# showlab/EgoVLP

Hardware: NVIDIA H100
Metric: clips/sec, 16-frame TimeSformer-B + DistilBERT + EgoNCE training step (higher is better)
Workload: dtype bf16

## Files before the change

egovlp_b200/csrc/attention.cu:

```cuda
#include <stdlib.h>

#include "common.cuh"
#include "egovlp_b200.h"

namespace egovlp {

bool space_attn_wgmma_supported(int N);
int space_attn_fwd_wgmma(const void* qkv, void* out, float* lse, float* cls_part, int B, int T, int N, int H,
                         cudaStream_t st);

namespace {

constexpr int HD = 64;
constexpr int ROW_BYTES = 128;
constexpr float LOG2E = 1.4426950408889634f;

struct Geom {
  int B, H, T, N, S, D;
  int mode;
  int PG;
  int G;
  int NP;
  int NPAD;
  int gsize;
};

__device__ __forceinline__ uint32_t sw_addr(uint32_t base, int row, int chunk) {
  return base + row * ROW_BYTES + ((chunk ^ (row & 7)) << 4);
}
__device__ __forceinline__ void ldsm_x4(uint32_t addr, uint32_t (&r)[4]) {
  asm volatile("ldmatrix.sync.aligned.m8n8.x4.shared.b16 {%0,%1,%2,%3}, [%4];"
               : "=r"(r[0]), "=r"(r[1]), "=r"(r[2]), "=r"(r[3]) : "r"(addr));
}
__device__ __forceinline__ void ldsm_x4_t(uint32_t addr, uint32_t (&r)[4]) {
  asm volatile("ldmatrix.sync.aligned.m8n8.x4.trans.shared.b16 {%0,%1,%2,%3}, [%4];"
               : "=r"(r[0]), "=r"(r[1]), "=r"(r[2]), "=r"(r[3]) : "r"(addr));
}
__device__ __forceinline__ void mma_bf16(float (&c)[4], const uint32_t (&a)[4], uint32_t b0, uint32_t b1) {
  asm volatile("mma.sync.aligned.m16n8k16.row.col.f32.bf16.bf16.f32 {%0,%1,%2,%3}, {%4,%5,%6,%7}, {%8,%9}, {%0,%1,%2,%3};"
               : "+f"(c[0]), "+f"(c[1]), "+f"(c[2]), "+f"(c[3])
               : "r"(a[0]), "r"(a[1]), "r"(a[2]), "r"(a[3]), "r"(b0), "r"(b1));
}
__device__ __forceinline__ void load_a_frag(uint32_t tile, int r0, int kk, int lane, uint32_t (&f)[4]) {
  ldsm_x4(sw_addr(tile, r0 + (lane & 7) + ((lane >> 3) & 1) * 8, kk * 2 + (lane >> 4)), f);
}
__device__ __forceinline__ void load_b_frag_nk(uint32_t tile, int n0, int kk, int lane, uint32_t (&f)[4]) {
  ldsm_x4(sw_addr(tile, n0 + (lane & 7) + (lane >> 4) * 8, kk * 2 + ((lane >> 3) & 1)), f);
}
__device__ __forceinline__ void load_b_frag_kn(uint32_t tile, int k0, int dp, int lane, uint32_t (&f)[4]) {
  ldsm_x4_t(sw_addr(tile, k0 + (lane & 7) + ((lane >> 3) & 1) * 8, dp * 2 + (lane >> 4)), f);
}

__device__ __forceinline__ int row_token(const Geom& G, int g, int r) {
  if (r == G.NP) return 0;
  if (r > G.NP) return -1;
  if (G.mode == 1) return 1 + g * G.N + r;
  const int j = r / G.T, f = r - j * G.T, n = g * G.PG + j;
  return n < G.N ? 1 + f * G.N + n : -1;
}

template <int RT>
__device__ __forceinline__ int row_token_x(const Geom& G, int g, int r, int sh) {
  if (RT == 0) return row_token(G, g, r);
  if (r == G.NP) return 0;
  if (r > G.NP) return -1;
  if (RT == 1) return 1 + g * G.N + r;
  const int n = g * G.PG + (r >> sh);
  return n < G.N ? 1 + (r & ((1 << sh) - 1)) * G.N + n : -1;
}

struct Smem {
  uint32_t q, k, v, dout;
  short* gid;
  float* lse;
  float* delta;
  uint32_t stage;
  uint32_t bar;
};

__device__ __forceinline__ bool pair_valid(int gq, int gk, bool first_group) {
  if (gq >= 0) return gk == gq || gk == -2;
  if (gq == -2) return gk >= 0 || (gk == -2 && first_group);
  return false;
}

__device__ __forceinline__ void tile_window(const Geom& G, int r0, int& lo, int& hi) {
  if (r0 <= G.NP && G.NP < r0 + 16) { lo = 0; hi = G.NP; return; }
  if (r0 > G.NP) { lo = 0; hi = 0; return; }
  lo = (r0 / G.gsize) * G.gsize;
  hi = min(G.NP, ((r0 + 15) / G.gsize + 1) * G.gsize);
}
__device__ __forceinline__ bool span_active(const Geom& G, int lo, int hi, int c0, int width) {
// ... 1038 lines not shown


}
}

using namespace egovlp;

extern "C" long long egovlp_divided_attn_workspace_floats(int B, int T, int N, int H, int mode) {
  Geom G;
  if (make_geom(G, B, T, N, H, mode)) return -1;
  return (long long)B * H * G.G * 4 * 66;
}

extern "C" int egovlp_divided_attn_fwd(const void* qkv, void* out, float* lse, float* cls_part, int B, int T, int N,
                                       int H, int mode, void* stream) {
  EGOVLP_CHECK_ARG(qkv && out && lse && cls_part, "divided_attn_fwd: null pointer");
  EGOVLP_CHECK_ARG(B > 0 && T > 0 && N > 0 && H > 0 && (mode == 0 || mode == 1), "divided_attn_fwd: bad shape");
  Geom G;
  if (make_geom(G, B, T, N, H, mode)) { set_last_error("divided_attn: unsupported geometry T=%d N=%d", T, N); return EGOVLP_ERR_UNSUPPORTED; }
  CUtensorMap tm;
  int rc = make_group_tmap(&tm, qkv, G, 3 * H);
  if (rc) return rc;
  cudaStream_t st = reinterpret_cast<cudaStream_t>(stream);
  const bf16* q = reinterpret_cast<const bf16*>(qkv);
  bf16* o = reinterpret_cast<bf16*>(out);
  const int grid = B * H * G.G;
#define LAUNCH_FWD(KERN, W, ...)                                                                              \
  do {                                                                                                        \
    const size_t smem = attn_smem_bytes(G, false, W, generic || mode == 1);                                   \
    EGOVLP_CHECK_CUDA(cudaFuncSetAttribute(KERN, cudaFuncAttributeMaxDynamicSharedMemorySize, (int)smem));    \
    KERN<<<grid, W * 32, smem, st>>>(tm, q, o, lse, cls_part, G, ##__VA_ARGS__);                              \
  } while (0)
  const bool generic = force_generic() || (mode == 0 && !time_fast_ok(G));
  if (!generic && mode == 1 && space_attn_wgmma_supported(N)) {
    rc = space_attn_fwd_wgmma(qkv, out, lse, cls_part, B, T, N, H, st);
    if (rc) return rc;
  } else if (generic) {
    if (G.NPAD > 128) LAUNCH_FWD((divided_attn_fwd_kernel<7, 2>), 7);
    else LAUNCH_FWD((divided_attn_fwd_kernel<4, 3>), 4);
  } else if (mode == 1) {
    if (G.NPAD > 128) LAUNCH_FWD((fast_attn_fwd_kernel<false, 7, 2>), 7, 0);
    else LAUNCH_FWD((fast_attn_fwd_kernel<false, 4, 3>), 4, 0);
  } else {
    LAUNCH_FWD((fast_attn_fwd_kernel<true, 4, 4>), 4, time_shift(G));
  }
#undef LAUNCH_FWD
  EGOVLP_CHECK_LAUNCH();
  const int BH = B * H;
  const int parts = (!generic && mode == 0) ? 4 : 1;
  cls_merge_kernel<<<(BH + 3) / 4, 128, 0, st>>>(cls_part, o, lse, BH, H, G.G * parts, G.S, G.D);
  EGOVLP_CHECK_LAUNCH();
  return EGOVLP_OK;
}

extern "C" int egovlp_divided_attn_bwd(const void* qkv, const void* out, const void* dout, const float* lse,
                                       void* dqkv, float* dcls_ws, int B, int T, int N, int H, int mode,
                                       float q_scale, void* stream) {
  EGOVLP_CHECK_ARG(qkv && out && dout && lse && dqkv && dcls_ws, "divided_attn_bwd: null pointer");
  EGOVLP_CHECK_ARG(B > 0 && T > 0 && N > 0 && H > 0 && (mode == 0 || mode == 1), "divided_attn_bwd: bad shape");
  Geom G;
  if (make_geom(G, B, T, N, H, mode)) { set_last_error("divided_attn: unsupported geometry T=%d N=%d", T, N); return EGOVLP_ERR_UNSUPPORTED; }
  CUtensorMap tmq, tmd;
  int rc = make_group_tmap(&tmq, qkv, G, 3 * H);
  if (rc) return rc;
  rc = make_group_tmap(&tmd, dout, G, H);
  if (rc) return rc;
  cudaStream_t st = reinterpret_cast<cudaStream_t>(stream);
  EGOVLP_CHECK_CUDA(cudaMemsetAsync(dcls_ws, 0, (size_t)B * H * 3 * HD * sizeof(float), st));
  const bf16* q = reinterpret_cast<const bf16*>(qkv);
  const bf16* o = reinterpret_cast<const bf16*>(out);
  const bf16* d_o = reinterpret_cast<const bf16*>(dout);
  bf16* dq = reinterpret_cast<bf16*>(dqkv);
  const int grid = B * H * G.G;
#define LAUNCH_BWD(KERN, W, ...)                                                                              \
  do {                                                                                                        \
    const size_t smem = attn_smem_bytes(G, true, W);                                                          \
    EGOVLP_CHECK_CUDA(cudaFuncSetAttribute(KERN, cudaFuncAttributeMaxDynamicSharedMemorySize, (int)smem));    \
    KERN<<<grid, W * 32, smem, st>>>(tmq, tmd, q, o, d_o, lse, dq, dcls_ws, q_scale, G, ##__VA_ARGS__);       \
  } while (0)
  const bool generic = force_generic() || (mode == 0 && !time_fast_ok(G));
  if (generic) {
    if (G.NPAD > 128) LAUNCH_BWD((divided_attn_bwd_kernel<7, 2>), 7);
    else LAUNCH_BWD((divided_attn_bwd_kernel<4, 3>), 4);
  } else if (mode == 1) {
    if (G.NPAD > 128) LAUNCH_BWD((fast_attn_bwd_kernel<false, 7, 2>), 7, 0);
    else LAUNCH_BWD((fast_attn_bwd_kernel<false, 4, 3>), 4, 0);
  } else {
    const char* we = getenv("EGOVLP_ATTN_TIME_BWD_WARPS");
    const bool w8 = we && we[0] == '8';
    if (w8) LAUNCH_BWD((fast_attn_bwd_kernel<true, 8, 2>), 8, time_shift(G));
    else LAUNCH_BWD((fast_attn_bwd_kernel<true, 4, 3>), 4, time_shift(G));
  }
#undef LAUNCH_BWD
  EGOVLP_CHECK_LAUNCH();
  const int n = B * H * 3 * HD;
  cls_grad_finalize_kernel<<<(n + 255) / 256, 256, 0, st>>>(dcls_ws, reinterpret_cast<bf16*>(dqkv), B, H, G.S, G.D, q_scale);
  EGOVLP_CHECK_LAUNCH();
  return EGOVLP_OK;
}
```

egovlp_b200/csrc/attention_wgmma.cu:

```cuda
#include <stdlib.h>

#include "common.cuh"
#include "egovlp_b200.h"

namespace egovlp {
namespace {

constexpr int HD = 64;
constexpr int ROWB = 128;
constexpr int QROWS = 256;
constexpr int KROWS = 208;
constexpr int Q_BYTES = QROWS * ROWB, KV_BYTES = KROWS * ROWB;
constexpr int SMEM_BYTES = Q_BYTES + 2 * KV_BYTES + 1024  + 64 ;
constexpr float LOG2E = 1.4426950408889634f;

struct SpaceGeom {
  int H, T, N, S, D;
};

__device__ __forceinline__ void wgmma_m64n208k16_ss(float (&d)[104], uint64_t adesc, uint64_t bdesc, int scale_d) {
  asm volatile(
      "{\n\t.reg .pred p;\n\t"
      "setp.ne.b32 p, %106, 0;\n\t"
      "wgmma.mma_async.sync.aligned.m64n208k16.f32.bf16.bf16 "
      "{%0,%1,%2,%3,%4,%5,%6,%7,%8,%9,%10,%11,%12,%13,%14,%15,%16,%17,%18,%19,%20,%21,%22,%23,%24,%25,%26,%27,%28,%29,%30,%31,"
      "%32,%33,%34,%35,%36,%37,%38,%39,%40,%41,%42,%43,%44,%45,%46,%47,%48,%49,%50,%51,%52,%53,%54,%55,%56,%57,%58,%59,%60,%61,%62,%63,"
      "%64,%65,%66,%67,%68,%69,%70,%71,%72,%73,%74,%75,%76,%77,%78,%79,%80,%81,%82,%83,%84,%85,%86,%87,%88,%89,%90,%91,%92,%93,%94,%95,"
      "%96,%97,%98,%99,%100,%101,%102,%103}, "
      "%104, %105, p, 1, 1, 0, 0;\n\t}"
      : "+f"(d[0]), "+f"(d[1]), "+f"(d[2]), "+f"(d[3]), "+f"(d[4]), "+f"(d[5]), "+f"(d[6]), "+f"(d[7]),
        "+f"(d[8]), "+f"(d[9]), "+f"(d[10]), "+f"(d[11]), "+f"(d[12]), "+f"(d[13]), "+f"(d[14]), "+f"(d[15]),
        "+f"(d[16]), "+f"(d[17]), "+f"(d[18]), "+f"(d[19]), "+f"(d[20]), "+f"(d[21]), "+f"(d[22]), "+f"(d[23]),
        "+f"(d[24]), "+f"(d[25]), "+f"(d[26]), "+f"(d[27]), "+f"(d[28]), "+f"(d[29]), "+f"(d[30]), "+f"(d[31]),
        "+f"(d[32]), "+f"(d[33]), "+f"(d[34]), "+f"(d[35]), "+f"(d[36]), "+f"(d[37]), "+f"(d[38]), "+f"(d[39]),
        "+f"(d[40]), "+f"(d[41]), "+f"(d[42]), "+f"(d[43]), "+f"(d[44]), "+f"(d[45]), "+f"(d[46]), "+f"(d[47]),
        "+f"(d[48]), "+f"(d[49]), "+f"(d[50]), "+f"(d[51]), "+f"(d[52]), "+f"(d[53]), "+f"(d[54]), "+f"(d[55]),
        "+f"(d[56]), "+f"(d[57]), "+f"(d[58]), "+f"(d[59]), "+f"(d[60]), "+f"(d[61]), "+f"(d[62]), "+f"(d[63]),
        "+f"(d[64]), "+f"(d[65]), "+f"(d[66]), "+f"(d[67]), "+f"(d[68]), "+f"(d[69]), "+f"(d[70]), "+f"(d[71]),
        "+f"(d[72]), "+f"(d[73]), "+f"(d[74]), "+f"(d[75]), "+f"(d[76]), "+f"(d[77]), "+f"(d[78]), "+f"(d[79]),
        "+f"(d[80]), "+f"(d[81]), "+f"(d[82]), "+f"(d[83]), "+f"(d[84]), "+f"(d[85]), "+f"(d[86]), "+f"(d[87]),
        "+f"(d[88]), "+f"(d[89]), "+f"(d[90]), "+f"(d[91]), "+f"(d[92]), "+f"(d[93]), "+f"(d[94]), "+f"(d[95]),
        "+f"(d[96]), "+f"(d[97]), "+f"(d[98]), "+f"(d[99]), "+f"(d[100]), "+f"(d[101]), "+f"(d[102]), "+f"(d[103])
      : "l"(adesc), "l"(bdesc), "r"(scale_d));
}
__device__ __forceinline__ void wgmma_m64n64k16_rs(float (&d)[32], uint32_t a0, uint32_t a1, uint32_t a2, uint32_t a3,
                                                  uint64_t bdesc, int scale_d) {
  asm volatile(
      "{\n\t.reg .pred p;\n\t"
      "setp.ne.b32 p, %37, 0;\n\t"
      "wgmma.mma_async.sync.aligned.m64n64k16.f32.bf16.bf16 "
      "{%0,%1,%2,%3,%4,%5,%6,%7,%8,%9,%10,%11,%12,%13,%14,%15,%16,%17,%18,%19,%20,%21,%22,%23,%24,%25,%26,%27,%28,%29,%30,%31}, "
      "{%32, %33, %34, %35}, %36, p, 1, 1, 1;\n\t}"
      : "+f"(d[0]), "+f"(d[1]), "+f"(d[2]), "+f"(d[3]), "+f"(d[4]), "+f"(d[5]), "+f"(d[6]), "+f"(d[7]),
        "+f"(d[8]), "+f"(d[9]), "+f"(d[10]), "+f"(d[11]), "+f"(d[12]), "+f"(d[13]), "+f"(d[14]), "+f"(d[15]),
        "+f"(d[16]), "+f"(d[17]), "+f"(d[18]), "+f"(d[19]), "+f"(d[20]), "+f"(d[21]), "+f"(d[22]), "+f"(d[23]),
        "+f"(d[24]), "+f"(d[25]), "+f"(d[26]), "+f"(d[27]), "+f"(d[28]), "+f"(d[29]), "+f"(d[30]), "+f"(d[31])
      : "r"(a0), "r"(a1), "r"(a2), "r"(a3), "l"(bdesc), "r"(scale_d));
}

__global__ void __launch_bounds__(256, 1)
space_attn_fwd_wgmma_kernel(const __grid_constant__ CUtensorMap tm_rows, const __grid_constant__ CUtensorMap tm_cls,
                            bf16* __restrict__ out, float* __restrict__ lse_out, float* __restrict__ cls_part, SpaceGeom G) {
  extern __shared__ uint8_t smem_raw[];
  const uint32_t base = (smem_u32(smem_raw) + 1023u) & ~1023u;
  uint8_t* gen = smem_raw + (base - smem_u32(smem_raw));
  const uint32_t sQ = base, sK = base + Q_BYTES, sV = sK + KV_BYTES, bar = sV + KV_BYTES;
  const int g = blockIdx.x;
  const int f = g % G.T, h = (g / G.T) % G.H, b = g / (G.T * G.H);
  const int NK = G.N + 1;

  for (int i = threadIdx.x; i < (Q_BYTES + 2 * KV_BYTES) / 16; i += blockDim.x)
    *reinterpret_cast<uint4*>(gen + 16 * i) = make_uint4(0, 0, 0, 0);
  fence_proxy_async_smem();
  if (threadIdx.x == 0) {
    mbar_init(bar, 1);
    fence_mbar_init();
  }
  __syncthreads();
  if (threadIdx.x == 0) {
    mbar_expect_tx(bar, 3u * (uint32_t)NK * ROWB);
#pragma unroll
    for (int w = 0; w < 3; ++w) {
      const uint32_t dst = w == 0 ? sQ : (w == 1 ? sK : sV);
      tma_load_4d(dst, &tm_rows, bar, 0, 1 + f * G.N, w * G.H + h, b);
      tma_load_4d(dst + G.N * ROWB, &tm_cls, bar, 0, 0, w * G.H + h, b);
    }
  }
  mbar_wait_nocall(bar, 0);

  const int wg = threadIdx.x >> 7, wq = (threadIdx.x >> 5) & 3, lane = threadIdx.x & 31;
  const int gq = lane >> 2, c = lane & 3;
  for (int t = wg; t < QROWS / 64; t += 2) {
    if (t * 64 > G.N) break;
    float s[KROWS / 2];
    wgmma_fence_regs(s);
    wgmma_fence();
#pragma unroll
    for (int kk = 0; kk < HD / 16; ++kk)
      wgmma_m64n208k16_ss(s, make_smem_desc_sw128(sQ + t * 64 * ROWB + kk * 32, 16, 1024),
                          make_smem_desc_sw128(sK + kk * 32, 16, 1024), kk > 0);
    wgmma_commit();
    wgmma_wait<0>();
    wgmma_fence_regs(s);
    const int r0 = t * 64 + wq * 16 + gq;
    float mx[2], sum[2];
#pragma unroll
    for (int h2 = 0; h2 < 2; ++h2) {
      const int vis = (r0 + 8 * h2 == G.N && f != 0) ? G.N : NK;
      float m = -INFINITY;
#pragma unroll
      for (int j = 0; j < KROWS / 8; ++j)
#pragma unroll
        for (int e = 0; e < 2; ++e) {
          float& v = s[4 * j + 2 * h2 + e];
          if (8 * j + 2 * c + e >= vis) v = -INFINITY;
          m = fmaxf(m, v);
        }
      m = fmaxf(m, __shfl_xor_sync(0xffffffffu, m, 1));
      mx[h2] = fmaxf(m, __shfl_xor_sync(0xffffffffu, m, 2));
    }
    uint32_t p[KROWS / 4];
#pragma unroll
    for (int h2 = 0; h2 < 2; ++h2) {
      const float nms = -mx[h2] * LOG2E;
      float acc = 0.f;
#pragma unroll
      for (int j = 0; j < KROWS / 8; ++j) {
        const float e0 = exp2f(fmaf(s[4 * j + 2 * h2], LOG2E, nms));
        const float e1 = exp2f(fmaf(s[4 * j + 2 * h2 + 1], LOG2E, nms));
        acc += e0 + e1;
        p[2 * j + h2] = pack_bf16x2(e0, e1);
      }
      acc += __shfl_xor_sync(0xffffffffu, acc, 1);
      sum[h2] = acc + __shfl_xor_sync(0xffffffffu, acc, 2);
    }
    float o[HD / 2];
    wgmma_fence_regs(o);
    wgmma_fence();
#pragma unroll
    for (int kk = 0; kk < KROWS / 16; ++kk)
      wgmma_m64n64k16_rs(o, p[4 * kk], p[4 * kk + 1], p[4 * kk + 2], p[4 * kk + 3],
                         make_smem_desc_sw128(sV + kk * 16 * ROWB, 8192, 1024), kk > 0);
    wgmma_commit();
    wgmma_wait<0>();
    wgmma_fence_regs(o);
#pragma unroll
    for (int h2 = 0; h2 < 2; ++h2) {
      const int row = r0 + 8 * h2;
      if (row < G.N) {
        const float inv = 1.f / sum[h2];
        const long long tok = (long long)b * G.S + 1 + f * G.N + row;
        bf16* dst = out + tok * G.D + h * HD + 2 * c;
#pragma unroll
        for (int j = 0; j < HD / 8; ++j)
          *reinterpret_cast<uint32_t*>(dst + 8 * j) = pack_bf16x2(o[4 * j + 2 * h2] * inv, o[4 * j + 2 * h2 + 1] * inv);
        if (c == 0) lse_out[((long long)(b * G.H + h)) * G.S + 1 + f * G.N + row] = mx[h2] + logf(sum[h2]);
      } else if (row == G.N) {
        float* dst = cls_part + (((long long)(b * G.H + h)) * G.T + f) * 66;
#pragma unroll
        for (int j = 0; j < HD / 8; ++j) {
          dst[8 * j + 2 * c] = o[4 * j + 2 * h2];
          dst[8 * j + 2 * c + 1] = o[4 * j + 2 * h2 + 1];
        }
        if (c == 0) { dst[64] = mx[h2]; dst[65] = sum[h2]; }
      }
    }
  }
}

}

bool space_attn_wgmma_supported(int N) {
  const char* e = getenv("EGOVLP_ATTN_TC");
  if (!(e && e[0] == '1')) return false;
  return N + 1 > 128 && N + 1 <= KROWS;
}

int space_attn_fwd_wgmma(const void* qkv, void* out, float* lse, float* cls_part, int B, int T, int N, int H,
                         cudaStream_t st) {
  SpaceGeom G;
  G.H = H; G.T = T; G.N = N; G.S = 1 + T * N; G.D = H * HD;
  const uint64_t W = 3ull * G.D;
  const uint64_t dims[4] = {HD, (uint64_t)G.S, (uint64_t)(3 * H), (uint64_t)B};
  const uint64_t strides[4] = {1, W, HD, (uint64_t)G.S * W};
  const uint32_t box_rows[4] = {HD, (uint32_t)N, 1, 1};
  const uint32_t box_cls[4] = {HD, 1, 1, 1};
  CUtensorMap tm_rows, tm_cls;
  int rc = make_tmap_nd_bf16(&tm_rows, qkv, 4, dims, strides, box_rows, true);
  if (rc) return rc;
  rc = make_tmap_nd_bf16(&tm_cls, qkv, 4, dims, strides, box_cls, true);
  if (rc) return rc;
  static bool attr = false;
  if (!attr) {
    EGOVLP_CHECK_CUDA(cudaFuncSetAttribute(space_attn_fwd_wgmma_kernel, cudaFuncAttributeMaxDynamicSharedMemorySize,
                                           SMEM_BYTES));
    attr = true;
  }
  space_attn_fwd_wgmma_kernel<<<B * H * T, 256, SMEM_BYTES, st>>>(tm_rows, tm_cls, reinterpret_cast<bf16*>(out), lse,
                                                                   cls_part, G);
  EGOVLP_CHECK_LAUNCH();
  return EGOVLP_OK;
}

}
```

egovlp_b200/csrc/common.cuh:

```cuda
#pragma once
#include <cuda.h>
#include <cuda_bf16.h>
#include <cuda_runtime.h>
#include <stdint.h>
#include <stdio.h>

#define EGOVLP_OK 0
#define EGOVLP_ERR_ARG (-1)
#define EGOVLP_ERR_CUDA (-2)
#define EGOVLP_ERR_UNSUPPORTED (-3)

namespace egovlp {

typedef __nv_bfloat16 bf16;

void set_last_error(const char* fmt, ...);

#define EGOVLP_CHECK_ARG(cond, ...)                                   \
  do {                                                                \
    if (!(cond)) {                                                    \
      ::egovlp::set_last_error(__VA_ARGS__);                          \
      return EGOVLP_ERR_ARG;                                          \
    }                                                                 \
  } while (0)
// ... 67 lines not shown
}
__device__ __forceinline__ unsigned long long dropout_key(unsigned long long seed, uint32_t site) {
  return seed ^ (0x9E3779B97F4A7C15ull * (unsigned long long)(site + 1));
}
__device__ __forceinline__ uint32_t dropout_threshold(float p) {
  const double t = (double)p * 4294967296.0;
  return t >= 4294967295.0 ? 0xFFFFFFFFu : (uint32_t)t;
}

__device__ __forceinline__ void mbar_init(uint32_t bar, uint32_t count) {
  asm volatile("mbarrier.init.shared::cta.b64 [%0], %1;" ::"r"(bar), "r"(count));
}
__device__ __forceinline__ void fence_mbar_init() {
  asm volatile("fence.mbarrier_init.release.cluster;" ::: "memory");
}
__device__ __forceinline__ void mbar_expect_tx(uint32_t bar, uint32_t bytes) {
  asm volatile("mbarrier.arrive.expect_tx.shared::cta.b64 _, [%0], %1;" ::"r"(bar), "r"(bytes) : "memory");
}
__device__ __forceinline__ void mbar_arrive(uint32_t bar) {
  asm volatile("mbarrier.arrive.shared::cta.b64 _, [%0];" ::"r"(bar) : "memory");
}
__device__ __forceinline__ uint32_t mbar_try_wait(uint32_t bar, uint32_t parity) {
  uint32_t ok;
  asm volatile(
      "{\n\t.reg .pred p;\n\t"
      "mbarrier.try_wait.parity.shared::cta.b64 p, [%1], %2;\n\t"
      "selp.u32 %0, 1, 0, p;\n\t}"
      : "=r"(ok)
      : "r"(bar), "r"(parity)
      : "memory");
  return ok;
}
__device__ __forceinline__ void mbar_wait(uint32_t bar, uint32_t parity) {
  if (mbar_try_wait(bar, parity)) return;
  const long long t0 = clock64();
  while (!mbar_try_wait(bar, parity)) {
    if (clock64() - t0 > 4000000000LL) {
      printf("egovlp: mbarrier timeout block %d thread %d bar %u parity %u\n", blockIdx.x, threadIdx.x, bar, parity);
      __trap();
    }
  }
}

__device__ __forceinline__ void mbar_wait_nocall(uint32_t bar, uint32_t parity) {
  if (mbar_try_wait(bar, parity)) return;
  const long long t0 = clock64();
  for (;;) {
#pragma unroll 1
    for (int i = 0; i < 1024; ++i)
      if (mbar_try_wait(bar, parity)) return;
    if (clock64() - t0 > 4000000000LL) __trap();
  }
}

__device__ __forceinline__ void tma_prefetch_desc(const CUtensorMap* m) {
  asm volatile("prefetch.tensormap [%0];" ::"l"(reinterpret_cast<uint64_t>(m)) : "memory");
}
__device__ __forceinline__ void tma_load_2d(uint32_t dst, const CUtensorMap* m, uint32_t bar, int c0, int c1) {
  asm volatile(
      "cp.async.bulk.tensor.2d.shared::cluster.global.mbarrier::complete_tx::bytes [%0], [%1, {%3, %4}], [%2];"
      ::"r"(dst), "l"(reinterpret_cast<uint64_t>(m)), "r"(bar), "r"(c0), "r"(c1)
      : "memory");
}
__device__ __forceinline__ void tma_load_3d(uint32_t dst, const CUtensorMap* m, uint32_t bar, int c0, int c1, int c2) {
  asm volatile(
      "cp.async.bulk.tensor.3d.shared::cluster.global.mbarrier::complete_tx::bytes [%0], [%1, {%3, %4, %5}], [%2];"
      ::"r"(dst), "l"(reinterpret_cast<uint64_t>(m)), "r"(bar), "r"(c0), "r"(c1), "r"(c2)
      : "memory");
}
__device__ __forceinline__ void tma_load_4d(uint32_t dst, const CUtensorMap* m, uint32_t bar, int c0, int c1, int c2,
                                            int c3) {
  asm volatile(
      "cp.async.bulk.tensor.4d.shared::cluster.global.mbarrier::complete_tx::bytes [%0], [%1, {%3, %4, %5, %6}], [%2];"
      ::"r"(dst), "l"(reinterpret_cast<uint64_t>(m)), "r"(bar), "r"(c0), "r"(c1), "r"(c2), "r"(c3)
      : "memory");
}
__device__ __forceinline__ void tma_load_5d(uint32_t dst, const CUtensorMap* m, uint32_t bar, int c0, int c1, int c2,
                                            int c3, int c4) {
  asm volatile(
      "cp.async.bulk.tensor.5d.shared::cluster.global.mbarrier::complete_tx::bytes [%0], [%1, {%3, %4, %5, %6, %7}], [%2];"
      ::"r"(dst), "l"(reinterpret_cast<uint64_t>(m)), "r"(bar), "r"(c0), "r"(c1), "r"(c2), "r"(c3), "r"(c4)
      : "memory");
}
__device__ __forceinline__ void tma_load_2d_multicast(uint32_t dst, const CUtensorMap* m, uint32_t bar, int c0, int c1,
                                                      uint16_t mask) {
  asm volatile(
      "cp.async.bulk.tensor.2d.shared::cluster.global.mbarrier::complete_tx::bytes.multicast::cluster"
      " [%0], [%1, {%3, %4}], [%2], %5;"
      ::"r"(dst), "l"(reinterpret_cast<uint64_t>(m)), "r"(bar), "r"(c0), "r"(c1), "h"(mask)
      : "memory");
}
__device__ __forceinline__ void fence_proxy_async_smem() {
  asm volatile("fence.proxy.async.shared::cta;" ::: "memory");
}
__device__ __forceinline__ void bulk_load_1d(uint32_t dst, const void* src, uint32_t bytes, uint32_t bar) {
  asm volatile("cp.async.bulk.shared::cluster.global.mbarrier::complete_tx::bytes [%0], [%1], %2, [%3];"
               ::"r"(dst), "l"(reinterpret_cast<uint64_t>(src)), "r"(bytes), "r"(bar)
               : "memory");
}
__device__ __forceinline__ void tma_store_2d(const CUtensorMap* m, uint32_t src, int c0, int c1) {
  asm volatile("cp.async.bulk.tensor.2d.global.shared::cta.bulk_group [%0, {%2, %3}], [%1];"
               ::"l"(reinterpret_cast<uint64_t>(m)), "r"(src), "r"(c0), "r"(c1)
               : "memory");
}
__device__ __forceinline__ void bulk_commit() { asm volatile("cp.async.bulk.commit_group;" ::: "memory"); }
template <int N>
__device__ __forceinline__ void bulk_wait_read() { asm volatile("cp.async.bulk.wait_group.read %0;" ::"n"(N) : "memory"); }
template <int N>
__device__ __forceinline__ void bulk_wait() { asm volatile("cp.async.bulk.wait_group %0;" ::"n"(N) : "memory"); }
__device__ __forceinline__ void named_bar_sync(int id, int count) {
  asm volatile("bar.sync %0, %1;" ::"r"(id), "r"(count) : "memory");
}

__device__ __forceinline__ uint32_t cluster_ctarank() {
  uint32_t r;
  asm volatile("mov.u32 %0, %%cluster_ctarank;" : "=r"(r));
  return r;
}
__device__ __forceinline__ void cluster_sync_all() {
  asm volatile("barrier.cluster.arrive.release.aligned;\n\tbarrier.cluster.wait.acquire.aligned;" ::: "memory");
}
__device__ __forceinline__ uint32_t mapa_shared(uint32_t addr, uint32_t cta_rank) {
  uint32_t r;
  asm volatile("mapa.shared::cluster.u32 %0, %1, %2;" : "=r"(r) : "r"(addr), "r"(cta_rank));
  return r;
}
__device__ __forceinline__ void mbar_arrive_cluster(uint32_t cluster_addr) {
  asm volatile("mbarrier.arrive.release.cluster.shared::cluster.b64 _, [%0];" ::"r"(cluster_addr) : "memory");
}

__device__ __forceinline__ void wgmma_fence() { asm volatile("wgmma.fence.sync.aligned;" ::: "memory"); }
__device__ __forceinline__ void wgmma_commit() { asm volatile("wgmma.commit_group.sync.aligned;" ::: "memory"); }
template <int N>
__device__ __forceinline__ void wgmma_wait() { asm volatile("wgmma.wait_group.sync.aligned %0;" ::"n"(N) : "memory"); }
template <int R>
__device__ __forceinline__ void wgmma_fence_regs(float (&d)[R]) {
#pragma unroll
  for (int i = 0; i < R; ++i) asm volatile("" : "+f"(d[i])::"memory");
}

__device__ __forceinline__ uint64_t make_smem_desc_sw128(uint32_t saddr, uint32_t lbo_bytes, uint32_t sbo_bytes) {
  uint64_t d = 0;
  d |= uint64_t((saddr >> 4) & 0x3FFF);
  d |= uint64_t((lbo_bytes >> 4) & 0x3FFF) << 16;
  d |= uint64_t((sbo_bytes >> 4) & 0x3FFF) << 32;
  d |= uint64_t(1) << 62;
  return d;
}

int make_tmap_2d_bf16(CUtensorMap* out, const void* base, uint64_t rows, uint64_t cols, uint64_t ld, uint32_t box_rows,
                      uint32_t box_cols);
int make_tmap_2d_f32(CUtensorMap* out, const void* base, uint64_t rows, uint64_t cols, uint64_t ld, uint32_t box_rows,
                     uint32_t box_cols);
int make_tmap_nd_bf16(CUtensorMap* out, const void* base, int rank, const uint64_t* dims, const uint64_t* strides,
                      const uint32_t* box, bool swizzle128);

}
```

Before: 174.5.

## Add persistent WGMMA space-attention backward kernel with TMA prefetch pipeline

Adds a Hopper wgmma-based backward kernel for the spatial (divided) attention. It is persistent, sized to the SM count, and loads Q/K/V/dO tiles with TMA, prefetching the next group into L2. It computes S and dP per key tile, builds dS in swizzled shared memory for the dQ GEMM, and overlaps the next group's loads with the current dQ computation. It is enabled by default whenever N+1 falls in (128,208]. The cost is a large shared-memory footprint, one CTA per SM, and atomic adds for the CLS gradient.

New measurement: 177.9, median of 6. +2.0%, better.

```diff
diff --git a/egovlp_b200/csrc/attention.cu b/egovlp_b200/csrc/attention.cu
--- a/egovlp_b200/csrc/attention.cu
+++ b/egovlp_b200/csrc/attention.cu
@@ -8,6 +8,9 @@
 bool space_attn_wgmma_supported(int N);
 int space_attn_fwd_wgmma(const void* qkv, void* out, float* lse, float* cls_part, int B, int T, int N, int H,
                          cudaStream_t st);
+bool space_attn_bwd_wgmma_supported(int N);
+int space_attn_bwd_wgmma(const void* qkv, const void* out, const void* dout, const float* lse, void* dqkv, float* dcls,
+                         int B, int T, int N, int H, float q_scale, cudaStream_t st);
 
 namespace {
 
@@ -1212,6 +1215,9 @@
   if (generic) {
     if (G.NPAD > 128) LAUNCH_BWD((divided_attn_bwd_kernel<7, 2>), 7);
     else LAUNCH_BWD((divided_attn_bwd_kernel<4, 3>), 4);
+  } else if (mode == 1 && space_attn_bwd_wgmma_supported(N)) {
+    rc = space_attn_bwd_wgmma(qkv, out, dout, lse, dqkv, dcls_ws, B, T, N, H, q_scale, st);
+    if (rc) return rc;
   } else if (mode == 1) {
     if (G.NPAD > 128) LAUNCH_BWD((fast_attn_bwd_kernel<false, 7, 2>), 7, 0);
     else LAUNCH_BWD((fast_attn_bwd_kernel<false, 4, 3>), 4, 0);
diff --git a/egovlp_b200/csrc/attention_wgmma.cu b/egovlp_b200/csrc/attention_wgmma.cu
--- a/egovlp_b200/csrc/attention_wgmma.cu
+++ b/egovlp_b200/csrc/attention_wgmma.cu
@@ -58,6 +58,53 @@
       : "r"(a0), "r"(a1), "r"(a2), "r"(a3), "l"(bdesc), "r"(scale_d));
 }
 
+__device__ __forceinline__ void wgmma_m64n112k16_ss(float (&d)[56], uint64_t adesc, uint64_t bdesc, int scale_d) {
+  asm volatile(
+      "{\n\t.reg .pred p;\n\t"
+      "setp.ne.b32 p, %58, 0;\n\t"
+      "wgmma.mma_async.sync.aligned.m64n112k16.f32.bf16.bf16 "
+      "{%0,%1,%2,%3,%4,%5,%6,%7,%8,%9,%10,%11,%12,%13,%14,%15,%16,%17,%18,%19,%20,%21,%22,%23,%24,%25,%26,%27,%28,%29,%30,%31,%32,%33,%34,%35,%36,%37,%38,%39,%40,%41,%42,%43,%44,%45,%46,%47,%48,%49,%50,%51,%52,%53,%54,%55}, "
+      "%56, %57, p, 1, 1, 0, 0;\n\t}"
+      : "+f"(d[0]), "+f"(d[1]), "+f"(d[2]), "+f"(d[3]), "+f"(d[4]), "+f"(d[5]), "+f"(d[6]), "+f"(d[7]),
+        "+f"(d[8]), "+f"(d[9]), "+f"(d[10]), "+f"(d[11]), "+f"(d[12]), "+f"(d[13]), "+f"(d[14]), "+f"(d[15]),
+        "+f"(d[16]), "+f"(d[17]), "+f"(d[18]), "+f"(d[19]), "+f"(d[20]), "+f"(d[21]), "+f"(d[22]), "+f"(d[23]),
+        "+f"(d[24]), "+f"(d[25]), "+f"(d[26]), "+f"(d[27]), "+f"(d[28]), "+f"(d[29]), "+f"(d[30]), "+f"(d[31]),
+        "+f"(d[32]), "+f"(d[33]), "+f"(d[34]), "+f"(d[35]), "+f"(d[36]), "+f"(d[37]), "+f"(d[38]), "+f"(d[39]),
+        "+f"(d[40]), "+f"(d[41]), "+f"(d[42]), "+f"(d[43]), "+f"(d[44]), "+f"(d[45]), "+f"(d[46]), "+f"(d[47]),
+        "+f"(d[48]), "+f"(d[49]), "+f"(d[50]), "+f"(d[51]), "+f"(d[52]), "+f"(d[53]), "+f"(d[54]), "+f"(d[55])
+      : "l"(adesc), "l"(bdesc), "r"(scale_d));
+}
+
+__device__ __forceinline__ void wgmma_m64n96k16_ss(float (&d)[48], uint64_t adesc, uint64_t bdesc, int scale_d) {
+  asm volatile(
+      "{\n\t.reg .pred p;\n\t"
+      "setp.ne.b32 p, %50, 0;\n\t"
+      "wgmma.mma_async.sync.aligned.m64n96k16.f32.bf16.bf16 "
+      "{%0,%1,%2,%3,%4,%5,%6,%7,%8,%9,%10,%11,%12,%13,%14,%15,%16,%17,%18,%19,%20,%21,%22,%23,%24,%25,%26,%27,%28,%29,%30,%31,%32,%33,%34,%35,%36,%37,%38,%39,%40,%41,%42,%43,%44,%45,%46,%47}, "
+      "%48, %49, p, 1, 1, 0, 0;\n\t}"
+      : "+f"(d[0]), "+f"(d[1]), "+f"(d[2]), "+f"(d[3]), "+f"(d[4]), "+f"(d[5]), "+f"(d[6]), "+f"(d[7]),
+        "+f"(d[8]), "+f"(d[9]), "+f"(d[10]), "+f"(d[11]), "+f"(d[12]), "+f"(d[13]), "+f"(d[14]), "+f"(d[15]),
+        "+f"(d[16]), "+f"(d[17]), "+f"(d[18]), "+f"(d[19]), "+f"(d[20]), "+f"(d[21]), "+f"(d[22]), "+f"(d[23]),
+        "+f"(d[24]), "+f"(d[25]), "+f"(d[26]), "+f"(d[27]), "+f"(d[28]), "+f"(d[29]), "+f"(d[30]), "+f"(d[31]),
+        "+f"(d[32]), "+f"(d[33]), "+f"(d[34]), "+f"(d[35]), "+f"(d[36]), "+f"(d[37]), "+f"(d[38]), "+f"(d[39]),
+        "+f"(d[40]), "+f"(d[41]), "+f"(d[42]), "+f"(d[43]), "+f"(d[44]), "+f"(d[45]), "+f"(d[46]), "+f"(d[47])
+      : "l"(adesc), "l"(bdesc), "r"(scale_d));
+}
+
+__device__ __forceinline__ void wgmma_m64n64k16_ss_tt(float (&d)[32], uint64_t adesc, uint64_t bdesc, int scale_d) {
+  asm volatile(
+      "{\n\t.reg .pred p;\n\t"
+      "setp.ne.b32 p, %34, 0;\n\t"
+      "wgmma.mma_async.sync.aligned.m64n64k16.f32.bf16.bf16 "
+      "{%0,%1,%2,%3,%4,%5,%6,%7,%8,%9,%10,%11,%12,%13,%14,%15,%16,%17,%18,%19,%20,%21,%22,%23,%24,%25,%26,%27,%28,%29,%30,%31}, "
+      "%32, %33, p, 1, 1, 1, 1;\n\t}"
+      : "+f"(d[0]), "+f"(d[1]), "+f"(d[2]), "+f"(d[3]), "+f"(d[4]), "+f"(d[5]), "+f"(d[6]), "+f"(d[7]),
+        "+f"(d[8]), "+f"(d[9]), "+f"(d[10]), "+f"(d[11]), "+f"(d[12]), "+f"(d[13]), "+f"(d[14]), "+f"(d[15]),
+        "+f"(d[16]), "+f"(d[17]), "+f"(d[18]), "+f"(d[19]), "+f"(d[20]), "+f"(d[21]), "+f"(d[22]), "+f"(d[23]),
+        "+f"(d[24]), "+f"(d[25]), "+f"(d[26]), "+f"(d[27]), "+f"(d[28]), "+f"(d[29]), "+f"(d[30]), "+f"(d[31])
+      : "l"(adesc), "l"(bdesc), "r"(scale_d));
+}
+
 __global__ void __launch_bounds__(256, 1)
 space_attn_fwd_wgmma_kernel(const __grid_constant__ CUtensorMap tm_rows, const __grid_constant__ CUtensorMap tm_cls,
                             bf16* __restrict__ out, float* __restrict__ lse_out, float* __restrict__ cls_part, SpaceGeom G) {
@@ -164,6 +211,247 @@
         }
         if (c == 0) { dst[64] = mx[h2]; dst[65] = sum[h2]; }
       }
+    }
+  }
+}
+
+constexpr int BQ_ROWS = 208;
+constexpr int BK_ROWS = 256;
+constexpr int QHALF = 112;
+constexpr int DS_SLAB = BQ_ROWS * ROWB;
+constexpr int B_OFF_V = BK_ROWS * ROWB, B_OFF_Q = 2 * BK_ROWS * ROWB, B_OFF_DO = B_OFF_Q + BQ_ROWS * ROWB,
+              B_OFF_DS = B_OFF_DO + BQ_ROWS * ROWB, B_OFF_LSE = B_OFF_DS + 4 * DS_SLAB,
+              B_OFF_DELTA = B_OFF_LSE + BQ_ROWS * 4, B_OFF_BAR = B_OFF_DELTA + BQ_ROWS * 4;
+constexpr int BWD_SMEM_BYTES = B_OFF_BAR + 16 + 1024 ;
+
+struct SpaceBwdGeom {
+  int H, T, N, S, D, groups;
+  float q_scale;
+};
+
+__device__ __forceinline__ void load_rows(uint32_t dst, const CUtensorMap* tm_rows, const CUtensorMap* tm_cls, uint32_t bar,
+                                          int col, int f, int b, int N) {
+  tma_load_4d(dst, tm_rows, bar, 0, 1 + f * N, col, b);
+  tma_load_4d(dst + N * ROWB, tm_cls, bar, 0, 0, col, b);
+}
+
+template <int NQ>
+__device__ __forceinline__ void wgmma_s_tile(float (&d)[NQ / 2], uint32_t a, uint32_t bq) {
+#pragma unroll
+  for (int kk = 0; kk < HD / 16; ++kk) {
+    const uint64_t ad = make_smem_desc_sw128(a + kk * 32, 16, 1024), bd = make_smem_desc_sw128(bq + kk * 32, 16, 1024);
+    if constexpr (NQ == 112) wgmma_m64n112k16_ss(d, ad, bd, kk > 0);
+    else wgmma_m64n96k16_ss(d, ad, bd, kk > 0);
+  }
+}
+
+template <int NQ>
+__device__ __forceinline__ void bwd_key_half(uint32_t sKt, uint32_t sVt, uint32_t sQ, uint32_t sDO, uint8_t* ds_gen,
+                                             const float* lse2, const float* delta, int q0, int key0, int c, int N,
+                                             bool cls_key_hidden, float (&dk)[32], float (&dv)[32]) {
+  float st[NQ / 2], dpt[NQ / 2];
+  wgmma_fence_regs(st);
+  wgmma_fence_regs(dpt);
+  wgmma_fence();
+  wgmma_s_tile<NQ>(st, sKt, sQ + q0 * ROWB);
+  wgmma_s_tile<NQ>(dpt, sVt, sDO + q0 * ROWB);
+  wgmma_commit();
+  wgmma_wait<0>();
+  wgmma_fence_regs(st);
+  wgmma_fence_regs(dpt);
+
+  uint32_t pf[NQ / 4], dsf[NQ / 4];
+#pragma unroll
+  for (int j = 0; j < NQ / 8; ++j) {
+    const int q = q0 + 8 * j + 2 * c;
+    const float2 l = *reinterpret_cast<const float2*>(lse2 + q);
+    const float2 dl = *reinterpret_cast<const float2*>(delta + q);
+#pragma unroll
+    for (int h2 = 0; h2 < 2; ++h2) {
+      const int key = key0 + 8 * h2;
+      float p0 = exp2f(fmaf(st[4 * j + 2 * h2], LOG2E, -l.x));
+      float p1 = exp2f(fmaf(st[4 * j + 2 * h2 + 1], LOG2E, -l.y));
+      if (key > N) { p0 = 0.f; p1 = 0.f; }
+      else if (key == N && cls_key_hidden) { p0 = q == N ? 0.f : p0; p1 = q + 1 == N ? 0.f : p1; }
+      const float d0 = p0 * (dpt[4 * j + 2 * h2] - dl.x), d1 = p1 * (dpt[4 * j + 2 * h2 + 1] - dl.y);
+      pf[2 * j + h2] = pack_bf16x2(p0, p1);
+      dsf[2 * j + h2] = pack_bf16x2(d0, d1);
+      if (key < BQ_ROWS)
+        *reinterpret_cast<uint32_t*>(ds_gen + (q >> 6) * DS_SLAB + key * ROWB + ((((q & 63) >> 3) ^ (key & 7)) << 4) +
+                                     (q & 7) * 2) = dsf[2 * j + h2];
+    }
+  }
+  wgmma_fence_regs(dk);
+  wgmma_fence_regs(dv);
+  wgmma_fence();
+#pragma unroll
+  for (int kk = 0; kk < NQ / 16; ++kk) {
+    wgmma_m64n64k16_rs(dv, pf[4 * kk], pf[4 * kk + 1], pf[4 * kk + 2], pf[4 * kk + 3],
+                       make_smem_desc_sw128(sDO + (q0 + 16 * kk) * ROWB, 8192, 1024), 1);
+    wgmma_m64n64k16_rs(dk, dsf[4 * kk], dsf[4 * kk + 1], dsf[4 * kk + 2], dsf[4 * kk + 3],
+                       make_smem_desc_sw128(sQ + (q0 + 16 * kk) * ROWB, 8192, 1024), 1);
+  }
+  wgmma_commit();
+  wgmma_wait<0>();
+  wgmma_fence_regs(dk);
+  wgmma_fence_regs(dv);
+}
+
+__device__ __forceinline__ void store_grad_rows(const float (&a)[32], int row0, int c, int N, float scale, bf16* dst_tok1,
+                                                long long ld, float* dcls_row) {
+#pragma unroll
+  for (int h2 = 0; h2 < 2; ++h2) {
+    const int r = row0 + 8 * h2;
+    if (r < N) {
+      bf16* dst = dst_tok1 + (long long)r * ld + 2 * c;
+#pragma unroll
+      for (int j = 0; j < HD / 8; ++j)
+        *reinterpret_cast<uint32_t*>(dst + 8 * j) = pack_bf16x2(a[4 * j + 2 * h2] * scale, a[4 * j + 2 * h2 + 1] * scale);
+    } else if (r == N) {
+#pragma unroll
+      for (int j = 0; j < HD / 8; ++j) {
+        atomicAdd(dcls_row + 8 * j + 2 * c, a[4 * j + 2 * h2]);
+        atomicAdd(dcls_row + 8 * j + 2 * c + 1, a[4 * j + 2 * h2 + 1]);
+      }
+    }
+  }
+}
+
+__global__ void __launch_bounds__(256, 1)
+space_attn_bwd_wgmma_kernel(const __grid_constant__ CUtensorMap tm_rows, const __grid_constant__ CUtensorMap tm_cls,
+                            const __grid_constant__ CUtensorMap tm_drows, const __grid_constant__ CUtensorMap tm_dcls,
+                            const __grid_constant__ CUtensorMap tm_orows, const bf16* __restrict__ out, const float* __restrict__ lse_in, bf16* __restrict__ dqkv,
+                            float* __restrict__ dcls, SpaceBwdGeom G) {
+  extern __shared__ uint8_t smem_raw[];
+  const uint32_t base = (smem_u32(smem_raw) + 1023u) & ~1023u;
+  uint8_t* gen = smem_raw + (base - smem_u32(smem_raw));
+  const uint32_t sK = base, sV = base + B_OFF_V, sQ = base + B_OFF_Q, sDO = base + B_OFF_DO, sDS = base + B_OFF_DS;
+  float* lse2 = reinterpret_cast<float*>(gen + B_OFF_LSE);
+  float* delta = reinterpret_cast<float*>(gen + B_OFF_DELTA);
+  const uint32_t bar_qvd = base + B_OFF_BAR, bar_k = bar_qvd + 8;
+  const int tid = threadIdx.x, wg = tid >> 7, wq = (tid >> 5) & 3, lane = tid & 31, gq = lane >> 2, c = lane & 3;
+  const int N = G.N, H = G.H;
+  const uint32_t qvd_bytes = 3u * (uint32_t)(N + 1) * ROWB, k_bytes = (uint32_t)(N + 1) * ROWB;
+
+  for (int i = tid; i < B_OFF_LSE / 16; i += blockDim.x) *reinterpret_cast<uint4*>(gen + 16 * i) = make_uint4(0, 0, 0, 0);
+  fence_proxy_async_smem();
+  if (tid == 0) {
+    mbar_init(bar_qvd, 1);
+    mbar_init(bar_k, 1);
+    fence_mbar_init();
+  }
+  __syncthreads();
+  auto issue_qvd = [&](int gi) {
+    const int h = gi % H, f = (gi / H) % G.T, b = gi / (H * G.T);
+    mbar_expect_tx(bar_qvd, qvd_bytes);
+    load_rows(sQ, &tm_rows, &tm_cls, bar_qvd, h, f, b, N);
+    load_rows(sV, &tm_rows, &tm_cls, bar_qvd, 2 * H + h, f, b, N);
+    load_rows(sDO, &tm_drows, &tm_dcls, bar_qvd, h, f, b, N);
+  };
+  auto issue_k = [&](int gi) {
+    const int h = gi % H, f = (gi / H) % G.T, b = gi / (H * G.T);
+    mbar_expect_tx(bar_k, k_bytes);
+    load_rows(sK, &tm_rows, &tm_cls, bar_k, H + h, f, b, N);
+  };
+  if (tid == 0 && (int)blockIdx.x < G.groups) {
+    issue_qvd(blockIdx.x);
+    issue_k(blockIdx.x);
+  }
+
+  constexpr int P0 = (BQ_ROWS + 31) / 32;
+  uint4 o_pre[P0];
+  float l_pre[P0];
+  auto load_o = [&](int gi) {
+    const int h = gi % H, f = (gi / H) % G.T, b = gi / (H * G.T);
+#pragma unroll
+    for (int i = 0; i < P0; ++i) {
+      const int r = (tid >> 3) + 32 * i;
+      const int tok = r < N ? 1 + f * N + r : 0;
+      o_pre[i] = __ldg(reinterpret_cast<const uint4*>(out + ((long long)b * G.S + tok) * G.D + h * HD + (tid & 7) * 8));
+      l_pre[i] = __ldg(lse_in + ((long long)b * H + h) * G.S + tok);
+    }
+  };
+  if ((int)blockIdx.x < G.groups) load_o(blockIdx.x);
+
+  uint32_t phase = 0;
+  for (int gi = blockIdx.x; gi < G.groups; gi += gridDim.x, phase ^= 1) {
+    const int h = gi % H, f = (gi / H) % G.T, b = gi / (H * G.T);
+    const long long bh = (long long)b * H + h;
+    const long long tok1 = (long long)b * G.S + 1 + (long long)f * N;
+    const int next = gi + gridDim.x;
+    if (tid == 0 && next < G.groups) {
+      const int hn = next % H, fn = (next / H) % G.T, bn = next / (H * G.T), r0 = 1 + fn * N;
+      tma_prefetch_l2_4d(&tm_rows, 0, r0, hn, bn);
+      tma_prefetch_l2_4d(&tm_rows, 0, r0, H + hn, bn);
+      tma_prefetch_l2_4d(&tm_rows, 0, r0, 2 * H + hn, bn);
+      tma_prefetch_l2_4d(&tm_drows, 0, r0, hn, bn);
+      tma_prefetch_l2_4d(&tm_orows, 0, r0, hn, bn);
+    }
+
+    mbar_wait_nocall(bar_qvd, phase);
+#pragma unroll
+    for (int i = 0; i < P0; ++i) {
+      const int r = (tid >> 3) + 32 * i, cc = tid & 7;
+      if (r >= BQ_ROWS) break;
+      const uint4 dv = *reinterpret_cast<const uint4*>(gen + B_OFF_DO + r * ROWB + ((cc ^ (r & 7)) << 4));
+      const uint32_t ou[4] = {o_pre[i].x, o_pre[i].y, o_pre[i].z, o_pre[i].w}, du[4] = {dv.x, dv.y, dv.z, dv.w};
+      float d = 0.f;
+#pragma unroll
+      for (int e = 0; e < 4; ++e) {
+        const float2 a = unpack_bf16x2(ou[e]), bb = unpack_bf16x2(du[e]);
+        d += a.x * bb.x + a.y * bb.y;
+      }
+      d += __shfl_xor_sync(0xffffffffu, d, 1);
+      d += __shfl_xor_sync(0xffffffffu, d, 2);
+      d += __shfl_xor_sync(0xffffffffu, d, 4);
+      if (cc == 0) {
+        delta[r] = r <= N ? d : 0.f;
+        lse2[r] = r <= N ? l_pre[i] * LOG2E : INFINITY;
+      }
+    }
+    mbar_wait_nocall(bar_k, phase);
+    __syncthreads();
+
+    for (int kt = wg; kt < BK_ROWS / 64; kt += 2) {
+      if (kt * 64 > N) break;
+      float dk[32], dv[32];
+#pragma unroll
+      for (int i = 0; i < 32; ++i) { dk[i] = 0.f; dv[i] = 0.f; }
+      const int key0 = kt * 64 + wq * 16 + gq;
+      const uint32_t sKt = sK + kt * 64 * ROWB, sVt = sV + kt * 64 * ROWB;
+      bwd_key_half<QHALF>(sKt, sVt, sQ, sDO, gen + B_OFF_DS, lse2, delta, 0, key0, c, N, f != 0, dk, dv);
+      bwd_key_half<BQ_ROWS - QHALF>(sKt, sVt, sQ, sDO, gen + B_OFF_DS, lse2, delta, QHALF, key0, c, N, f != 0, dk, dv);
+      bf16* dst = dqkv + tok1 * 3 * G.D + h * HD;
+      store_grad_rows(dk, kt * 64 + wq * 16 + gq, c, N, 1.f, dst + G.D, 3 * G.D, dcls + (bh * 3 + 1) * HD);
+      store_grad_rows(dv, kt * 64 + wq * 16 + gq, c, N, 1.f, dst + 2 * G.D, 3 * G.D, dcls + (bh * 3 + 2) * HD);
+    }
+    fence_proxy_async_smem();
+    __syncthreads();
+    if (tid == 0 && next < G.groups) issue_qvd(next);
+    if (next < G.groups) load_o(next);
+
+    {
+      float dq0[32], dq1[32];
+      wgmma_fence_regs(dq0);
+      wgmma_fence_regs(dq1);
+      wgmma_fence();
+#pragma unroll
+      for (int kk = 0; kk < BQ_ROWS / 16; ++kk) {
+        const uint64_t bd = make_smem_desc_sw128(sK + kk * 16 * ROWB, 8192, 1024);
+        wgmma_m64n64k16_ss_tt(dq0, make_smem_desc_sw128(sDS + wg * DS_SLAB + kk * 16 * ROWB, 8192, 1024), bd, kk > 0);
+        wgmma_m64n64k16_ss_tt(dq1, make_smem_desc_sw128(sDS + (wg + 2) * DS_SLAB + kk * 16 * ROWB, 8192, 1024), bd,
+                              kk > 0);
+      }
+      wgmma_commit();
+      wgmma_wait<0>();
+      wgmma_fence_regs(dq0);
+      wgmma_fence_regs(dq1);
+      named_bar_sync(1, 256);
+      if (tid == 0 && next < G.groups) issue_k(next);
+      bf16* dst = dqkv + tok1 * 3 * G.D + h * HD;
+      float* dcq = dcls + (bh * 3 + 0) * HD;
+      store_grad_rows(dq0, wg * 64 + wq * 16 + gq, c, N, G.q_scale, dst, 3 * G.D, dcq);
+      store_grad_rows(dq1, (wg + 2) * 64 + wq * 16 + gq, c, N, G.q_scale, dst, 3 * G.D, dcq);
     }
   }
 }
@@ -202,4 +490,42 @@
   return EGOVLP_OK;
 }
 
-}
+bool space_attn_bwd_wgmma_supported(int N) {
+  const char* e = getenv("EGOVLP_ATTN_SPACE_BWD");
+  if (e && e[0] == 'm') return false;
+  return N + 1 > 128 && N + 1 <= BQ_ROWS;
+}
+
+int space_attn_bwd_wgmma(const void* qkv, const void* out, const void* dout, const float* lse, void* dqkv, float* dcls,
+                         int B, int T, int N, int H, float q_scale, cudaStream_t st) {
+  SpaceBwdGeom G;
+  G.H = H; G.T = T; G.N = N; G.S = 1 + T * N; G.D = H * HD; G.groups = B * H * T; G.q_scale = q_scale;
+  const uint64_t W = 3ull * G.D;
+  const uint64_t dims[4] = {HD, (uint64_t)G.S, (uint64_t)(3 * H), (uint64_t)B};
+  const uint64_t strides[4] = {1, W, HD, (uint64_t)G.S * W};
+  const uint64_t ddims[4] = {HD, (uint64_t)G.S, (uint64_t)H, (uint64_t)B};
+  const uint64_t dstrides[4] = {1, (uint64_t)G.D, HD, (uint64_t)G.S * G.D};
+  const uint32_t box_rows[4] = {HD, (uint32_t)N, 1, 1};
+  const uint32_t box_cls[4] = {HD, 1, 1, 1};
+  CUtensorMap tm_rows, tm_cls, tm_drows, tm_dcls, tm_orows;
+  int rc = make_tmap_nd_bf16(&tm_rows, qkv, 4, dims, strides, box_rows, true);
+  if (!rc) rc = make_tmap_nd_bf16(&tm_cls, qkv, 4, dims, strides, box_cls, true);
+  if (!rc) rc = make_tmap_nd_bf16(&tm_drows, dout, 4, ddims, dstrides, box_rows, true);
+  if (!rc) rc = make_tmap_nd_bf16(&tm_dcls, dout, 4, ddims, dstrides, box_cls, true);
+  if (!rc) rc = make_tmap_nd_bf16(&tm_orows, out, 4, ddims, dstrides, box_rows, true);
+  if (rc) return rc;
+  static bool attr = false;
+  if (!attr) {
+    EGOVLP_CHECK_CUDA(cudaFuncSetAttribute(space_attn_bwd_wgmma_kernel, cudaFuncAttributeMaxDynamicSharedMemorySize,
+                                           BWD_SMEM_BYTES));
+    attr = true;
+  }
+  const int grid = G.groups < num_sms() ? G.groups : num_sms();
+  space_attn_bwd_wgmma_kernel<<<grid, 256, BWD_SMEM_BYTES, st>>>(tm_rows, tm_cls, tm_drows, tm_dcls, tm_orows,
+                                                                  reinterpret_cast<const bf16*>(out), lse,
+                                                                  reinterpret_cast<bf16*>(dqkv), dcls, G);
+  EGOVLP_CHECK_LAUNCH();
+  return EGOVLP_OK;
+}
+
+}
diff --git a/egovlp_b200/csrc/common.cuh b/egovlp_b200/csrc/common.cuh
--- a/egovlp_b200/csrc/common.cuh
+++ b/egovlp_b200/csrc/common.cuh
@@ -173,6 +173,11 @@
       ::"r"(dst), "l"(reinterpret_cast<uint64_t>(m)), "r"(bar), "r"(c0), "r"(c1), "r"(c2), "r"(c3), "r"(c4)
       : "memory");
 }
+__device__ __forceinline__ void tma_prefetch_l2_4d(const CUtensorMap* m, int c0, int c1, int c2, int c3) {
+  asm volatile("cp.async.bulk.prefetch.tensor.4d.L2.global.tile [%0, {%1, %2, %3, %4}];"
+               ::"l"(reinterpret_cast<uint64_t>(m)), "r"(c0), "r"(c1), "r"(c2), "r"(c3)
+               : "memory");
+}
 __device__ __forceinline__ void tma_load_2d_multicast(uint32_t dst, const CUtensorMap* m, uint32_t bar, int c0, int c1,
                                                       uint16_t mask) {
   asm volatile(
```
